# a-ludi/dentist

Hardware: AMD Instinct MI355X
Metric: gap-bases closed/sec (higher is better)
Workload: dtype u8

## Files before the change

dentist_amd/_lib.py:

```python
import ctypes
import os
import weakref

import numpy as np

_HERE = os.path.dirname(os.path.abspath(__file__))


def lib_path():
    return os.environ.get("DH_DEV_LIB") or os.path.join(_HERE, "libdentist_hip.so")


class DhError(RuntimeError):
    def __init__(self, code, msg):
        super().__init__(f"libdentist_hip error {code}: {msg}")
        self.code = code


class AlignOpts(ctypes.Structure):
    _fields_ = [(n, ctypes.c_int32) for n in (
        "k", "hmin", "band_shift", "tspace", "min_len", "pen", "xdrop", "max_err_ppm", "max_cand",
        "max_la", "tcap", "strands", "skip_self", "dmax", "width", "kmer_mod", "algo")]


# ... 29 lines not shown
    "contig_left", "status", "nreads", "ref_read", "ref_read_id", "crop_left", "crop_right", "left_aepos",
    "right_abpos", "ins_begin", "ins_end", "comp", "cons_len", "left_diffs", "right_diffs", "join")]
    + [("cons_off", "<i8"), ("contig_right", "<i4"), ("pad", "<i4")])

EXACT_HIT_DTYPE = np.dtype([("query", "<i4"), ("ref", "<i4"), ("begin", "<i8"), ("end", "<i8"), ("complement", "<i4"),
                            ("pad", "<i4")])

LA_DTYPE = np.dtype([("tlen", "<i4"), ("diffs", "<i4"), ("abpos", "<i4"), ("bbpos", "<i4"),
                     ("aepos", "<i4"), ("bepos", "<i4"), ("flags", "<u4"), ("aread", "<i4"),
                     ("bread", "<i4"), ("pad", "<i4"), ("toff", "<i8")])

SYMBOLS = [
    "dh_last_error", "dh_abi_version", "dh_ctx_create", "dh_ctx_destroy", "dh_ctx_sync",
    "dh_default_align_opts", "dh_db_create", "dh_db_destroy", "dh_db_drop_cache", "dh_db_nreads",
    "dh_db_total_bases", "dh_la_set_destroy", "dh_la_set_count", "dh_la_set_trace_len",
    "dh_la_set_records", "dh_la_set_trace", "dh_la_set_tspace", "dh_get_align_stats", "dh_get_cum_stats", "dh_get_mjoin_counts", "dh_get_join_counts", "dh_join_hit_capacity",
    "dh_ctx_release_scratch",
    "dh_align_db",
    "dh_las_write", "dh_las_read", "dh_default_process_opts", "dh_collect_spanning", "dh_pileups_destroy",
    "dh_pileups_count", "dh_pileups_get", "dh_process_pileups", "dh_insertions_destroy",
    "dh_insertions_count", "dh_insertions_records", "dh_insertions_bases", "dh_insertions_bases_len",
    "dh_get_process_stats", "dh_dazz_create_dam", "dh_dazz_create_db", "dh_dazz_split", "dh_dazz_open",
    "dh_dazz_close", "dh_dazz_nreads", "dh_dazz_first_id", "dh_dazz_bases", "dh_dazz_offsets",
    "dh_dazz_origin", "dh_dazz_fpulse", "dh_dazz_header", "dh_dazz_read_mask", "dh_dazz_write_mask",
    "dh_db_set_mask", "dh_output_fasta", "dh_tile_qv", "dh_consensus", "dh_las_merge",
    "dh_collect_candidates", "dh_pileups_create", "dh_pileups_select", "dh_align_db_block", "dh_la_set_merge",
    "dh_crop_pileups", "dh_cropped_create", "dh_cropped_destroy", "dh_cropped_npiles", "dh_cropped_records",
    "dh_cropped_nreads", "dh_cropped_pile", "dh_cropped_entry", "dh_cropped_read_id", "dh_cropped_offsets",
    "dh_cropped_bases", "dh_process_cropped", "dh_translate_trace_point", "dh_db_dust", "dh_db_get_mask",
    "dh_dazz_write_track", "dh_dazz_read_track", "dh_dazz_remove", "dh_dazz_flags",
    "dh_pileupdb_write", "dh_pileupdb_read", "dh_insertiondb_write", "dh_insertiondb_read", "dh_insertiondb_merge", "dh_chaindb_destroy",
# ... 255 lines not shown
        lib().dh_ctx_release_scratch.argtypes = [ctypes.c_void_p]
        _check(lib().dh_ctx_release_scratch(self._h))

    def mjoin_counts(self, reset=False):
        out = (ctypes.c_int64 * 2)()
        lib().dh_get_mjoin_counts.argtypes = [ctypes.c_void_p, ctypes.c_void_p, ctypes.c_int32]
        _check(lib().dh_get_mjoin_counts(self._h, out, int(reset)))
        return int(out[0]), int(out[1])

    def join_counts(self, reset=False):
        out = (ctypes.c_int64 * 4)()
        lib().dh_get_join_counts.argtypes = [ctypes.c_void_p, ctypes.c_void_p, ctypes.c_int32]
        _check(lib().dh_get_join_counts(self._h, out, int(reset)))
        return tuple(int(x) for x in out)

    def cum_stats(self, reset=False):
        st = CumStats()
        _check(lib().dh_get_cum_stats(self._h, ctypes.byref(st), int(reset)))
        return st

    def remap_skipping_reads(self, contigs, reads, contig_ids, read_ids, opts, allowance):
        ci = np.ascontiguousarray(contig_ids, dtype=np.int32)
        ri = np.ascontiguousarray(read_ids, dtype=np.int32)
        h = ctypes.c_void_p()
        L = lib()
        L.dh_remap_skipping_reads.argtypes = [ctypes.c_void_p, ctypes.c_void_p, ctypes.c_void_p, ctypes.c_void_p, ctypes.c_int32,
                                              ctypes.c_void_p, ctypes.c_int32, ctypes.c_void_p, ctypes.c_int32,
                                              ctypes.POINTER(ctypes.c_void_p)]
        _check(L.dh_remap_skipping_reads(self._h, contigs._h, reads._h, ci.ctypes.data, len(ci), ri.ctypes.data, len(ri),
                                         ctypes.byref(opts), int(allowance), ctypes.byref(h)))
# ... 1422 lines not shown
```

dentist_amd/csrc/dh_align.cpp:

```cpp
#include <chrono>
#include <cmath>
#include <cstdio>
#include <cstdlib>
#include <cstring>
#include <numeric>
#include <functional>
#include <memory>
#include <mutex>
#include <thread>

#include "dh_internal.h"
#include "dh_join.h"
#include "dh_mjoin.h"
#include "dh_tile.h"
#include "dh_parallel.h"

#define fail dh_fail

#ifdef DH_SEED_PROF
extern "C" void dhk_seed_prof_dump();
extern "C" void dhk_join_prof_dump();
extern "C" void dhk_tile_prof_dump();
#endif


extern "C" int dh_align_db(dh_ctx *ctx, dh_db *A, dh_db *B, const dh_align_opts *opts,
                           int32_t want_best, dh_la_set **out)
{
// ... 158 lines not shown
    }
    ~Tasks() { join(); }
};

struct AlignRun {
    dh_ctx *ctx;
    dh_db *A, *B;
    const dh_align_opts &o;
    int32_t first, count, want_best, want_sorted;
    const ChunkHook *hook;
    hipStream_t st;
    int32_t near_ppm;
    std::unique_ptr<dh_la_set> res, res2;
    Tasks tasks;
    dh_align_stats stats = {};
    bool tiled, use_join = false, use_mj = false, db_copies = false, want_packed = false, dual = false, sym_tiled = false,
         keep_dev = false;
    int64_t nitems_total, item_first, item_end;
    int32_t sepv = 0, chunk = 0, cn = 0, nbmax = 0, trmax = 0, per_wave = 0, poolcap = 0, nslots = 0, tile_waves = 0;
    int cap = 0;
    double dens = 0;
    int64_t mj_min_bases = 0;
    DhOpts dopt;
    IndexView iv;
    DbView av, bv;
    JoinView jv = {};
    int64_t join_hits = 0;
    float ms_join = 0;
    unsigned int jhist[4] = {0, 0, 0, 0};
    DhCand *d_cand = nullptr;
    int32_t *d_ncand = nullptr, *d_nhits = nullptr, *d_status = nullptr, *d_cdj = nullptr, *d_ovf = nullptr, *d_regs = nullptr;
// ... 375 lines not shown
    }
    HIPCHK(hipEventElapsedTime(&r.ms_join, ctx->ev[6], ctx->ev[7]));
    if (getenv("DH_TRACE"))
        fprintf(stderr, "[join] hit buffer %lld (%.1f MB), %lld hits, %d attempt(s); %.4f hits per base per read of depth from now on\n",
                (long long)ctx->join_first_cap, (double)ctx->join_first_cap * sizeof(uint64_t) / 1048576.0, (long long)r.join_hits,
                attempt + 1, ctx->join_hit_rate);
    if (!r.use_join) {
        if (getenv("DH_TRACE")) fprintf(stderr, "[join] a slice overflowed its table: falling back to the k-mer directory\n");
        HIPCHK(hipMemsetAsync(r.d_status, 0, sizeof(int32_t), st));
        if (int rc = dh_build_index(A, o.k, r.sepv, o.kmer_mod, false)) return rc;
        r.iv = index_view(A);
    }
    return DH_OK;
}

static int plan_seeds(AlignRun &r)
{
    dh_db *A = r.A, *B = r.B;
    const dh_align_opts &o = r.o;
    r.dens = (double)A->ix.n * std::max(1, o.kmer_mod) / std::pow(4.0, o.k) / std::max(1, A->ngroups);
    const double exp_hits = (double)B->max_len / std::max(1, o.kmer_mod) * (2.0 * r.dens + 0.1);
    int cap = 1024;
    while (cap < 16384 && exp_hits * 1.5 >= cap) cap *= 2;
    if (A == B) {
        cap = 1024;
        while (cap < 8192 && 0.6 * B->max_len > cap) cap *= 2;
    }
    if (r.use_join) {
        const unsigned int tol = (unsigned int)(0.3 * B->n);
        cap = r.jhist[0] <= tol ? 2048 : (r.jhist[1] <= tol ? 4096 : (r.jhist[2] <= tol ? 8192 : 16384));
    }
    if (const char *e = getenv("DH_SEED_CAP")) cap = atoi(e);
    r.cap = cap;
    r.use_mj = !r.use_join && A != B && !A->d_group && A->ngroups == 1 && !B->d_group && o.k >= MJ_MINK && o.k <= MJ_MAXK &&
               o.skip_self == 0 && r.want_packed && A->ix.n > 0 && A->ix.n < (1ll << 28) && !getenv("DH_NO_MJOIN");
    r.mj_min_bases = 64ll << 20;
    if (const char *e = getenv("DH_MJOIN_MIN")) r.mj_min_bases = atoll(e);
    if (r.use_mj && !A->ix.d_bitmap) {
        int32_t nbbits = std::min(MJ_MAXBITS, std::min(2 * o.k, std::max(MJ_PBITS + 5, dh_ceil_log2((uint64_t)A->ix.n) + 4)));
        const size_t words = (size_t)1 << (nbbits - 5);
        HIPCHK(dh_dev_alloc(&A->ix.d_bitmap, sizeof(uint32_t) * words));
        HIPCHK(dhk_memset(r.st, A->ix.d_bitmap, 0, sizeof(uint32_t) * words));
        dhk_mj_bitmap(r.st, A->ix.d_ent, A->ix.n, o.k, nbbits, A->ix.d_bitmap);
        HIPCHK(hipGetLastError());
        A->ix.nbbits = nbbits;
    }
    return DH_OK;
}

static int plan_mj_chunk(AlignRun &r, AlignChunk &c)
{
    dh_ctx *ctx = r.ctx;
    const dh_db *A = r.A, *B = r.B;
    const dh_align_opts &o = r.o;
    MjView &mv = c.mv;
    const int32_t cr0 = (int32_t)(c.item0 >> 1), cr1 = (int32_t)((c.item0 + c.ni) >> 1);
    const int64_t cb0 = B->h_off[(size_t)cr0], cb1 = B->h_off[(size_t)cr1];
    if (!r.use_mj || r.mj_skip_chunk || cb1 - cb0 < r.mj_min_bases || cb1 - cb0 >= (1ll << 40)) return DH_OK;
    mv.c0 = cb0;
    mv.c1 = cb1;
// ... 106 lines not shown
        SCR(SLOT_FSCR, d_fscr, (size_t)ctx->ncu * DH_SEED_FSCR_BLOCKS_PER_CU * DH_SEED_FSCR_WORDS)
    JoinView jv_mj = {};
    bool mj_chunk = false;
    if (c.mj_planned && !c.cc.has_n) {
        const MjView &mv = c.mv;
        HIPCHK(dhk_memset(st, mv.segtab, 0, sizeof(unsigned long long) * (size_t)(mv.r1 - mv.r0) * mv.nseg));
        dhk_mj_run(st, r.bv, r.iv, r.dopt, mv, ctx->ncu);
        HIPCHK(hipGetLastError());
        jv_mj.segtab = (uint64_t *)mv.segtab;
        jv_mj.hits = mv.rhits;
        jv_mj.status = r.d_status;
        jv_mj.ns_fixed = mv.nseg;
        jv_mj.read0 = mv.r0;
        mj_chunk = true;
    }
    const bool jn = r.use_join || mj_chunk;
    const JoinView &jvx = mj_chunk ? jv_mj : r.jv;
    const int tier_max = getenv("DH_SEED_NO16K") ? 8192 : 16384;
    const double kmers_per_read = (double)(B->h_off[(size_t)((item0 + ni) >> 1)] - B->h_off[(size_t)(item0 >> 1)]) /
                                  std::max(1, ni / 2) / std::max(1, o.kmer_mod);
    const double mean_hits = kmers_per_read * (2.0 * r.dens + 0.075);
    const bool wave_tier = mj_chunk && ctx->seed_wave_tier && 1.5 * mean_hits <= 512.0 && !getenv("DH_SEED_NO_WAVE_TIER");
    int capj = std::min(std::max(r.cap, 2048), tier_max);
    if (mj_chunk) {
        capj = 2048;
        while (capj < tier_max && 1.5 * mean_hits > capj) capj *= 2;
        if (wave_tier) capj = 512;
    }
    if (jn && capj > 4096) SCR(SLOT_FSCR, d_fscr, (size_t)ctx->ncu * DH_SEED_FSCR_BLOCKS_PER_CU * (capj > 8192 ? DH_SEED_FSCR_WORDS16 : DH_SEED_FSCR_WORDS))
    if (jn)
        dhk_seed_join(st, capj, r.bv, r.iv, r.dopt, jvx, (int32_t)item0, ni, c.candbase, c.ncandbase, c.nhitsbase, r.d_status,
                      r.d_queue + 1, ctx->ncu, d_fscr, nullptr, 0);
    else
        dhk_seed(st, r.cap, r.bv, r.iv, r.dopt, (int32_t)item0, ni, c.candbase, c.ncandbase, c.nhitsbase, r.d_status,
                 r.d_queue + 1, ctx->ncu, d_fscr);
    HIPCHK(hipGetLastError());
    int32_t status = 0;
    unsigned long long sm[4] = {0, 0, 0, 0};
    dhk_seed_summary(st, r.d_ncand, r.d_nhits, ni, r.d_summary);
// ... 42 lines not shown
        ctx->seed_wave_tier = 0;
        if (getenv("DH_TRACE"))
            fprintf(stderr, "[seeds] %zu of %d reads overflow the wavefront-per-read tier: not used by this context any more\n", big.size(), ni / 2);
    }
    size_t redo_all = (size_t)ni / 50 + 8;
    if (r.cap >= 8192) redo_all = (size_t)ni / 4;
    if (const char *e = getenv("DH_SEED_BIG_PCT")) redo_all = (size_t)((double)ni * atof(e) / 200.0);
    if (getenv("DH_TRACE") && !big.empty())
        fprintf(stderr, "[seeds] cap %d: %zu of %d reads overflow (whole chunk again above %zu)\n", r.cap, big.size(), ni / 2, redo_all);
    if (!jn && big.size() > redo_all && r.cap < 16384) {
        r.cap *= 2;
        *redo = true;
        return DH_OK;
    }
    if (mj_chunk) ctx->mj_chunks++;
    r.mj_skip_chunk = false;
    if (jn && capj < tier_max && !big.empty()) {
        std::vector<int32_t> huge;
        int32_t gcap2 = 0;
        for (int tier = capj < 2048 ? 2048 : 8192; tier <= tier_max; tier = tier < 8192 ? 8192 : tier * 2) {
            if (tier <= capj) continue;
            std::vector<int32_t> mid;
            huge.clear();
            gcap2 = 0;
            for (int32_t rd : big) {
                const size_t it = (size_t)(2 * (int64_t)rd - item0);
                const int32_t nh = r.h_nhits[it] + r.h_nhits[it + 1];
                if (nh <= tier)
                    mid.push_back(rd);
                else {
// ... 523 lines not shown
```

dentist_amd/csrc/dh_api.cpp:

```cpp
#include <cstring>

#include "dh_internal.h"

static_assert(sizeof(dh_align_opts) == sizeof(DhOpts), "opts layout");
static_assert(sizeof(dh_la) == sizeof(DhLa), "la layout");
static_assert(sizeof(dh_la) == 48, "la size");

static thread_local std::string g_err;

int dh_fail(int code, const std::string &msg)
{
    g_err = msg;
    return code;
}
#define fail dh_fail

extern "C" const char *dh_last_error(void) { return g_err.c_str(); }
extern "C" int32_t dh_abi_version(void) { return 4; }



extern "C" int dh_ctx_create(int32_t device, void *stream, dh_ctx **out)
{
    if (!out) return fail(DH_EINVAL, "dh_ctx_create: out is NULL");
// ... 104 lines not shown
{
    if (!c) return fail(DH_EINVAL, "ctx is NULL");
    HIPCHK(hipStreamSynchronize(c->stream));
    return DH_OK;
}

extern "C" int dh_get_mjoin_counts(dh_ctx *c, int64_t *out2, int32_t reset)
{
    if (!c || !out2) return fail(DH_EINVAL, "dh_get_mjoin_counts: NULL");
    out2[0] = c->mj_chunks;
    out2[1] = c->mj_fallbacks;
    if (reset) c->mj_chunks = c->mj_fallbacks = 0;
    return DH_OK;
}

extern "C" int dh_get_join_counts(dh_ctx *c, int64_t *out4, int32_t reset)
{
    if (!c || !out4) return fail(DH_EINVAL, "dh_get_join_counts: NULL");
    out4[0] = c->join_launches;
    out4[1] = c->join_reruns;
    out4[2] = c->join_last_hits;
    out4[3] = c->join_first_cap;
    if (reset) c->join_launches = c->join_reruns = c->join_last_hits = c->join_first_cap = 0;
    return DH_OK;
}

extern "C" int dh_get_align_stats(dh_ctx *c, dh_align_stats *out)
{
    if (!c || !out) return fail(DH_EINVAL, "dh_get_align_stats: NULL");
    *out = c->stats;
// ... 32 lines not shown
```

dentist_amd/csrc/dh_db.cpp:

```cpp
#include <cmath>
#include <cstdlib>

#include "dh_internal.h"

#define fail dh_fail


int dh_alloc_bases(hipStream_t st, int64_t total, uint8_t **alloc, uint8_t **base, bool pads_only)
{
    const size_t nb = (size_t)std::max<int64_t>(total, 0) + 2 * DB_PAD;
    HIPCHK(dh_dev_alloc(alloc, nb));
    if (pads_only) {
        HIPCHK(hipMemsetAsync(*alloc, 4, DB_PAD, st));
        HIPCHK(hipMemsetAsync(*alloc + nb - DB_PAD, 4, DB_PAD, st));
    } else
        HIPCHK(dhk_memset(st, *alloc, 4, nb));
    *base = *alloc + DB_PAD;
    return DH_OK;
}



extern "C" int dh_db_create(dh_ctx *ctx, const uint8_t *bases, const int64_t *off, int32_t n,
                            const int32_t *group, dh_db **out)
// ... 459 lines not shown
    HIPCHK(hipStreamSynchronize(ctx->stream));
    if (total != (unsigned long long)nent || total >= (1ull << 32) - 16)
        return fail(DH_EOVERFLOW, "index: more than 2^32 indexed k-mers (32-bit bucket offsets); raise kmer_mod");
    ix.n = (int64_t)nent;
    HIPCHK(dh_dev_alloc(&ix.d_ent, sizeof(ulonglong2) * (size_t)std::max<int64_t>(ix.n, 1)));
    if (gi_slices > 0)
        dhk_group_index(ctx->stream, 1, av, d_tiles, d_gtile, A->ngroups, gi_slices, gi_slice, k, kmer_mod, ix.shift,
                        ix.d_dir, ix.d_ent, ix.d_goff);
    else
        dhk_kmer_pass(ctx->stream, 1, av, d_tiles, (int32_t)tiles.size(), k, kmer_mod, ix.shift, ix.d_dir, ix.d_ent,
                      ix.d_goff);
    HIPCHK(hipGetLastError());
    HIPCHK(dh_dev_alloc(&ix.d_fat, sizeof(ulonglong2) * (size_t)nb));
    dhk_fat_dir(ctx->stream, ix.d_dir, ix.d_ent, nb, ix.d_fat);
    HIPCHK(hipGetLastError());
    HIPCHK(hipStreamSynchronize(ctx->stream));
    dh_dev_free(d_tiles);
    dh_dev_free(d_sums);
    dh_dev_free(ix.d_dir_alloc);
    ix.d_dir_alloc = ix.d_dir = nullptr;
    A->has_ix = true;
    return DH_OK;
}
```

dentist_amd/csrc/dh_internal.h:

```cpp
#ifndef DH_INTERNAL_H
#define DH_INTERNAL_H

#include "../../include/dentist_hip.h"

#include <hip/hip_runtime.h>

#include <algorithm>
#include <string>
#include <new>
#include <utility>
#include <vector>

#include "dh_device.h"

#define DB_PAD 64
#define PK_PAD 128

hipError_t dh_dev_alloc(void **p, size_t bytes);
void dh_dev_free(void *p);
void dh_dev_trim();
template <typename T>
inline hipError_t dh_dev_alloc(T **p, size_t bytes)
{
    return dh_dev_alloc((void **)p, bytes);
// ... 34 lines not shown
            return dh_fail(DH_EHIP, std::string(#expr) + ": " + hipGetErrorString(e_));          \
    } while (0)

enum DhSlot : int {
    SLOT_STATUS,
    SLOT_CAND, SLOT_NCAND, SLOT_NHITS, SLOT_NLA, SLOT_NTR, SLOT_POOL, SLOT_CDJ, SLOT_QUEUE, SLOT_LA, SLOT_TRSLOTS,
    SLOT_COUNTERS, SLOT_SUMS, SLOT_SUMMARY, SLOT_OVF, SLOT_REGS, SLOT_COLD, SLOT_LAOUT, SLOT_TROUT,
    SLOT_FSCR, SLOT_MID_LIST, SLOT_BIG_LIST, SLOT_BIG_HITS,
    SLOT_UNITS, SLOT_CANDOFF, SLOT_RECLIST, SLOT_RECCUR,
    SLOT_LA2, SLOT_TRSLOTS2, SLOT_NLA2, SLOT_NTR2, SLOT_A_PLANES, SLOT_A_RC_PLANES, SLOT_B_PK2, SLOT_B_RC_PK2, SLOT_LAOUT2,
    SLOT_TROUT2,
    SLOT_CHUNK_RC, SLOT_CHUNK_PK, SLOT_CHUNK_RCPK,
    SLOT_JOIN_BLOB, SLOT_JOIN_PSUB, SLOT_JOIN_ENTRIES, SLOT_JOIN_SEGTAB, SLOT_JOIN_CURSOR, SLOT_JOIN_HITS,
    SLOT_MJ_ENT, SLOT_MJ_SEGOFF, SLOT_MJ_TILE_N, SLOT_MJ_TILE_R, SLOT_MJ_SEG, SLOT_MJ_HSEG, SLOT_MJ_HITS, SLOT_MJ_RHITS,
    SLOT_MJ_SEGTAB, SLOT_MJ_CTR,
    SLOT_PR_VOFF, SLOT_PR_VOTES, SLOT_PR_OUT, SLOT_PR_STATUS, SLOT_PR_STAGE, SLOT_PR_SEGS, SLOT_PR_DECISIONS, SLOT_PR_CDIFF,
    SLOT_COMM_SEND, SLOT_COMM_RECV,
    SLOT_EP_TILES, SLOT_EP_DM, SLOT_EP_OW, SLOT_EP_RES, SLOT_EP_GEN_TILES, SLOT_EP_GEN_DM, SLOT_EP_GEN_OW, SLOT_EP_GEN_OFF,
    SLOT_EP_GEN_RES, SLOT_EP_COPY, SLOT_EP_OPS,
    SLOT_TR_RECS, SLOT_TR_BOUND, SLOT_TR_PAIRS, SLOT_TR_STATUS,
    SLOT_NW_REF, SLOT_NW_QRY, SLOT_NW_PAIRS, SLOT_NW_DM, SLOT_NW_OW, SLOT_NW_RES, SLOT_NW_COPY, SLOT_NW_OPS,
    SLOT_NWA_REF, SLOT_NWA_QRY, SLOT_NWA_PAIRS, SLOT_NWA_DM, SLOT_NWA_OW, SLOT_NWA_RES, SLOT_NWA_COPY, SLOT_NWA_OPS,
    SLOT_LOC_TEXT, SLOT_LOC_STARTS, SLOT_LOC_PW, SLOT_LOC_PATS, SLOT_LOC_MEMB, SLOT_LOC_TABLE, SLOT_LOC_BITMAP, SLOT_LOC_SHORTS,
    SLOT_LOC_CANDS, SLOT_LOC_COUNTER, SLOT_LOC_UNITS,
    DH_SLOT_COUNT
};
enum { DH_STW_STATUS = 0, DH_STW_PACK = 1, DH_STW_PACK_RC = 2, DH_STW_COUNT = 4 };
static_assert(DH_STW_PACK_RC == DH_STW_PACK + 1, "chunk_copies clears the two flag words with one memset");

#define DH_JOIN_HIT_RATE0 0.0128
#define DH_JOIN_HIT_MARGIN 1.5
#define DH_JOIN_HIT_MEM_FRACTION 0.25

struct dh_ctx {
    int device = 0;
    hipStream_t stream = nullptr;
    bool own_stream = false;
    int ncu = 0;
    hipEvent_t ev[8] = {};
    hipStream_t cstream = nullptr;
    hipEvent_t cev[4] = {};
    dh_align_stats stats = {};
    dh_cum_stats cum = {};
    double mj_hit_frac = 0.2;
    int seed_wave_tier = 1;
    int64_t mj_chunks = 0, mj_fallbacks = 0;
    double join_hit_rate = DH_JOIN_HIT_RATE0;
    int64_t join_launches = 0, join_reruns = 0, join_last_hits = 0, join_first_cap = 0;
    int32_t near_best_ppm = -1;
    dh_ctx *sub[3] = {nullptr, nullptr, nullptr};
    struct Arena {
        void *p = nullptr;
        size_t cap = 0;
    } arena[DH_SLOT_COUNT];
};
int dh_scratch(dh_ctx *ctx, DhSlot id, size_t bytes, void **out);
int dh_db_set_pflags(struct dh_db *db, const uint8_t *flags);

struct dh_index {
    uint32_t *d_dir = nullptr, *d_dir_alloc = nullptr;
    ulonglong2 *d_fat = nullptr;
    ulonglong2 *d_ent = nullptr;
    int64_t *d_goff = nullptr;
    int32_t *d_page_seq = nullptr;
    int64_t n = 0;
    int32_t k = 0, sepv = 0, shift = 0, pbits = 0, na = 0, kmer_mod = 1;
    uint32_t *d_bitmap = nullptr;
    int32_t nbbits = 0;
    bool light = false;
    void release()
    {
        dh_dev_free(d_dir_alloc);
        d_dir_alloc = nullptr;
        dh_dev_free(d_ent);
        dh_dev_free(d_goff);
        dh_dev_free(d_fat);
        d_fat = nullptr;
        dh_dev_free(d_page_seq);
        d_page_seq = nullptr;
        dh_dev_free(d_bitmap);
        d_bitmap = nullptr;
        nbbits = 0;
        d_dir = nullptr;
        d_ent = nullptr;
        d_goff = nullptr;
    }
// ... 127 lines not shown
```

dentist_amd/csrc/dh_process.cpp:

```cpp
#include <array>
#include <chrono>
#include <thread>
#include <cstdio>
#include <cstdlib>
#include <cstring>
#include <map>
#include <mutex>
#include <numeric>

#include "dh_internal.h"
#include "dh_parallel.h"

extern "C" {
void dhk_gather_slices(hipStream_t st, const uint8_t *src, const int64_t *src_off, const int32_t *sidx,
                       const int32_t *sbeg, const int64_t *dst_off, int32_t n, int32_t max_len,
                       uint8_t *dst);
void dhk_gather_parts(hipStream_t st, const uint8_t *src0, const int64_t *off0, const uint8_t *src1,
                      const int64_t *off1, const void *parts, int32_t n, int32_t max_len, uint8_t *dst);
void dhk_gather_ranges16(hipStream_t st, const uint16_t *src, const int64_t *desc, int32_t n, uint16_t *dst);
void dhk_tile_qv(hipStream_t st, const DhLa *las, const uint16_t *trace, const int32_t *la_first,
                 const int64_t *roff, int32_t nreads, int32_t tspace, const int32_t *cov, int32_t maxtiles,
                 uint8_t *qv);
void dhk_pile_funnel(hipStream_t st, DhLa *las, const uint32_t *item_off, int32_t nreads, const int64_t *roff,
                     int32_t max_err_ppm, int32_t tsp, int32_t *la_first, int32_t *live, int32_t *status);
// ... 1676 lines not shown
        rcs[0] = dh_fail(DH_EINVAL, std::string("dh_process_pileups: the first part of the batch failed: ") + e.what());
    }
    for (std::thread &w : workers) w.join();
    for (int32_t k = 1; k < nparts; k++) {
        dh_cum_stats &a = ctx->cum, &b = ctx->sub[k - 1]->cum;
        a.ms_index += b.ms_index; a.ms_seed += b.ms_seed; a.ms_wave += b.ms_wave; a.ms_gather += b.ms_gather;
        a.wave_launches += b.wave_launches; a.wave_cells += b.wave_cells; a.alignments += b.alignments; a.las += b.las;
        a.aligned_bp += b.aligned_bp; a.trace_values += b.trace_values; a.hits += b.hits; a.b_bases += b.b_bases;
        b = dh_cum_stats();
        dh_ctx *sc = ctx->sub[k - 1];
        ctx->join_launches += sc->join_launches;
        ctx->join_reruns += sc->join_reruns;
        ctx->join_last_hits += sc->join_last_hits;
        ctx->join_first_cap += sc->join_first_cap;
        sc->join_launches = sc->join_reruns = sc->join_last_hits = sc->join_first_cap = 0;
    }
    for (int32_t k = 0; k < nparts; k++)
        if (rcs[(size_t)k]) {
            for (dh_insertions *r : res) dh_insertions_destroy(r);
            if (k == 0) return rcs[0];
            return dh_fail(rcs[(size_t)k], msgs[(size_t)k].empty() ? "dh_process_pileups: a concurrent part of the batch failed" : msgs[(size_t)k]);
        }
    for (int32_t k = 1; k < nparts; k++) {
        for (int i = 0; i < 7; i++) g_pstats.ms[i] = std::max(g_pstats.ms[i], sts[(size_t)k].ms[i]);
        for (int i = 0; i < 3; i++) g_pstats.counters[i] += sts[(size_t)k].counters[i];
        for (int i = 0; i < 4; i++) g_pstats.work[i] += sts[(size_t)k].work[i];
    }
    dh_insertions *r0 = res[0];
    for (int32_t k = 1; k < nparts; k++) {
        dh_insertions *r1 = res[(size_t)k];
// ... 1267 lines not shown
```

include/dentist_hip.h:

```cpp
#ifndef DENTIST_HIP_H
#define DENTIST_HIP_H

#include <stddef.h>
#include <stdint.h>

#ifdef __cplusplus
extern "C" {
#endif

#define DH_OK 0
#define DH_EINVAL (-1)
#define DH_ENODEV (-2)
#define DH_EHIP (-3)
#define DH_EOVERFLOW (-4)
#define DH_EIO (-5)
#define DH_ENOMEM (-6)

const char *dh_last_error(void);
int32_t dh_abi_version(void);

typedef struct dh_ctx dh_ctx;
int dh_ctx_create(int32_t device, void *stream, dh_ctx **out);
void dh_ctx_destroy(dh_ctx *ctx);
int dh_ctx_sync(dh_ctx *ctx);
// ... 57 lines not shown
    float ms_index, ms_seed, ms_wave, ms_gather, ms_total;
    int32_t wave_launches;
    int32_t overflow_items;
    int64_t big_items;
} dh_align_stats;
int dh_get_align_stats(dh_ctx *ctx, dh_align_stats *out);

typedef struct {
    double ms_index, ms_seed, ms_wave, ms_gather;
    int64_t wave_launches, wave_cells, alignments, las, aligned_bp, trace_values, hits, b_bases;
} dh_cum_stats;
int dh_get_cum_stats(dh_ctx *ctx, dh_cum_stats *out, int32_t reset);
int dh_ctx_release_scratch(dh_ctx *ctx);
int dh_get_mjoin_counts(dh_ctx *ctx, int64_t *out2, int32_t reset);
int dh_get_join_counts(dh_ctx *ctx, int64_t *out4, int32_t reset);
int64_t dh_join_hit_capacity(const int64_t *bases, const int32_t *reads, int32_t ngroups, int32_t skip_self, double rate,
                             int64_t free_bytes);

int dh_align_db(dh_ctx *ctx, dh_db *A, dh_db *B, const dh_align_opts *opts, int32_t select_best,
                dh_la_set **out);
void dh_set_near_best(int32_t ppm);
int dh_ctx_set_near_best(dh_ctx *ctx, int32_t ppm);

int dh_align_db_block(dh_ctx *ctx, dh_db *A, dh_db *B, int32_t first, int32_t count,
                      const dh_align_opts *opts, int32_t select_best, dh_la_set **out);
int dh_align_db_transposed(dh_ctx *ctx, dh_db *A, dh_db *B, const dh_align_opts *opts, int32_t want_best,
                           dh_la_set **out, dh_la_set **out_transposed);
int dh_la_set_merge(const dh_la_set *const *sets, int32_t nsets, dh_la_set **out);

int dh_las_write(const char *path, const dh_la *las, int64_t n, const uint16_t *trace,
// ... 391 lines not shown
```

Baseline: 2.369 million.

## Add shared-memory hash-table join for grouped seed lookup

Adds a new seeding path (table join) for reads grouped by contig. For each group it builds a shared-memory hash table of the group's index k-mers, and each wave of B reads probes that table with count and write passes, producing segmented hit lists. It replaces the generic k-mer directory lookup when limits on group size, k and read length hold, and falls back otherwise. The cost is an extra count pass, a host sync per chunk to size the hit buffer with possible reruns, and an extra group-offset kernel at index build.

```diff
diff --git a/dentist_amd/_lib.py b/dentist_amd/_lib.py
--- a/dentist_amd/_lib.py
+++ b/dentist_amd/_lib.py
@@ -67,7 +67,7 @@
     "dh_last_error", "dh_abi_version", "dh_ctx_create", "dh_ctx_destroy", "dh_ctx_sync",
     "dh_default_align_opts", "dh_db_create", "dh_db_destroy", "dh_db_drop_cache", "dh_db_nreads",
     "dh_db_total_bases", "dh_la_set_destroy", "dh_la_set_count", "dh_la_set_trace_len",
-    "dh_la_set_records", "dh_la_set_trace", "dh_la_set_tspace", "dh_get_align_stats", "dh_get_cum_stats", "dh_get_mjoin_counts", "dh_get_join_counts", "dh_join_hit_capacity",
+    "dh_la_set_records", "dh_la_set_trace", "dh_la_set_tspace", "dh_get_align_stats", "dh_get_cum_stats", "dh_get_mjoin_counts", "dh_get_join_counts", "dh_get_tjoin_counts", "dh_join_hit_capacity",
     "dh_ctx_release_scratch",
     "dh_align_db",
     "dh_las_write", "dh_las_read", "dh_default_process_opts", "dh_collect_spanning", "dh_pileups_destroy",
@@ -353,6 +353,12 @@
         _check(lib().dh_get_join_counts(self._h, out, int(reset)))
         return tuple(int(x) for x in out)
 
+    def tjoin_counts(self, reset=False):
+        out = (ctypes.c_int64 * 4)()
+        lib().dh_get_tjoin_counts.argtypes = [ctypes.c_void_p, ctypes.c_void_p, ctypes.c_int32]
+        _check(lib().dh_get_tjoin_counts(self._h, out, int(reset)))
+        return tuple(int(x) for x in out)
+
     def cum_stats(self, reset=False):
         st = CumStats()
         _check(lib().dh_get_cum_stats(self._h, ctypes.byref(st), int(reset)))
diff --git a/dentist_amd/csrc/dh_align.cpp b/dentist_amd/csrc/dh_align.cpp
--- a/dentist_amd/csrc/dh_align.cpp
+++ b/dentist_amd/csrc/dh_align.cpp
@@ -12,6 +12,7 @@
 #include "dh_internal.h"
 #include "dh_join.h"
 #include "dh_mjoin.h"
+#include "dh_tjoin.h"
 #include "dh_tile.h"
 #include "dh_parallel.h"
 
@@ -200,7 +201,7 @@
     std::unique_ptr<dh_la_set> res, res2;
     Tasks tasks;
     dh_align_stats stats = {};
-    bool tiled, use_join = false, use_mj = false, db_copies = false, want_packed = false, dual = false, sym_tiled = false,
+    bool tiled, use_join = false, use_mj = false, use_tj = false, db_copies = false, want_packed = false, dual = false, sym_tiled = false,
          keep_dev = false;
     int64_t nitems_total, item_first, item_end;
     int32_t sepv = 0, chunk = 0, cn = 0, nbmax = 0, trmax = 0, per_wave = 0, poolcap = 0, nslots = 0, tile_waves = 0;
@@ -606,6 +607,11 @@
     return DH_OK;
 }
 
+static void ctx_count_tj_fallback(dh_ctx *ctx)
+{
+    ctx->tj_fallbacks++;
+    if (getenv("DH_TRACE")) fprintf(stderr, "[tjoin] a limit of the table join is not met: this call keeps the k-mer directory\n");
+}
 static int plan_seeds(AlignRun &r)
 {
     dh_db *A = r.A, *B = r.B;
@@ -636,6 +642,17 @@
         dhk_mj_bitmap(r.st, A->ix.d_ent, A->ix.n, o.k, nbbits, A->ix.d_bitmap);
         HIPCHK(hipGetLastError());
         A->ix.nbbits = nbbits;
+    }
+    if (!r.use_join && A != B && A->d_group && !getenv("DH_NO_TJOIN")) {
+        int64_t tcap_ent = TJ_CAP;
+        if (const char *e = getenv("DH_TJOIN_CAP")) tcap_ent = std::max<int64_t>(0, std::min<int64_t>(TJ_CAP, atoll(e)));
+        r.use_tj = B->d_group && o.k <= TJ_MAXK && o.skip_self == 0 && A->ix.d_gent &&
+                   A->ix.max_gent <= tcap_ent && A->ix.n < (1ll << 31) && B->max_len < (1 << 24);
+        if (!r.use_tj) ctx_count_tj_fallback(r.ctx);
+        if (r.use_tj) {
+            r.ctx->tj_calls++;
+            r.ctx->tj_last_hits = 0;
+        }
     }
     return DH_OK;
 }
@@ -772,15 +789,82 @@
         jv_mj.read0 = mv.r0;
         mj_chunk = true;
     }
-    const bool jn = r.use_join || mj_chunk;
-    const JoinView &jvx = mj_chunk ? jv_mj : r.jv;
+    JoinView jv_tj = {};
+    bool tj_chunk = false;
+    unsigned long long tj_hits = 0;
+    if (r.use_tj) {
+        const int32_t cr0 = (int32_t)(item0 >> 1), cr1 = (int32_t)((item0 + ni) >> 1);
+        std::vector<int4> units;
+        for (int32_t rd = cr0; rd < cr1;) {
+            const int32_t g = B->h_group[(size_t)rd];
+            int32_t e = rd + 1;
+            while (e < cr1 && e - rd < TJ_RUN && B->h_group[(size_t)e] == g) e++;
+            units.push_back(int4{g, rd, e, 0});
+            rd = e;
+        }
+        const int64_t cbases = B->h_off[(size_t)cr1] - B->h_off[(size_t)cr0];
+        int64_t hcap = (int64_t)(1.25 * ctx->tj_hit_rate * (double)cbases) + 4096;
+        if (const char *e = getenv("DH_TJOIN_HITCAP")) hcap = std::max<int64_t>(1, atoll(e));
+        TjView tv = {};
+        int4 *d_units;
+        uint32_t *d_tjctr;
+        SCR(SLOT_TJ_UNITS, d_units, units.size())
+        SCR(SLOT_TJ_SEGTAB, tv.segtab, (size_t)(cr1 - cr0))
+        SCR(SLOT_TJ_CTR, d_tjctr, 4)
+        HIPCHK(hipMemcpyAsync(d_units, units.data(), sizeof(int4) * units.size(), hipMemcpyHostToDevice, st));
+        tv.gent = r.A->ix.d_gent;
+        tv.ngroups = r.A->ngroups;
+        tv.units = d_units;
+        tv.nunits = (int32_t)units.size();
+        tv.read0 = cr0;
+        tv.cursor = (unsigned long long *)d_tjctr;
+        tv.queue = d_tjctr + 2;
+        tv.status = r.d_status;
+        int32_t tst = 0;
+        for (int attempt = 0;; attempt++) {
+            SCR(SLOT_TJ_HITS, tv.hits, (size_t)hcap)
+            tv.hits_cap = hcap;
+            HIPCHK(hipMemsetAsync(d_tjctr, 0, 4 * sizeof(uint32_t), st));
+            dhk_tjoin(st, r.bv, r.iv, r.dopt, tv, ctx->ncu);
+            HIPCHK(hipGetLastError());
+            HIPCHK(hipMemcpyAsync(&tj_hits, tv.cursor, sizeof(tj_hits), hipMemcpyDeviceToHost, st));
+            HIPCHK(hipMemcpyAsync(&tst, r.d_status, sizeof(int32_t), hipMemcpyDeviceToHost, st));
+            HIPCHK(hipStreamSynchronize(st));
+            if (!(tst & DH_ST_TJ_HITCAP)) break;
+            if (attempt > 0) return fail(DH_EOVERFLOW, "table join: the hit buffer sized by the count pass was too small");
+            tst &= ~DH_ST_TJ_HITCAP;
+            HIPCHK(hipMemcpyAsync(r.d_status, &tst, sizeof(int32_t), hipMemcpyHostToDevice, st));
+            if (getenv("DH_TRACE")) fprintf(stderr, "[tjoin] hit buffer of %lld too small for %llu hits: run again\n", (long long)hcap, tj_hits);
+            hcap = (int64_t)tj_hits;
+            ctx->tj_reruns++;
+        }
+        if (cbases > 0) ctx->tj_hit_rate = std::max(DH_TJ_HIT_RATE0, (double)tj_hits / (double)cbases);
+        if (tst & DH_ST_TJ_OVERFLOW) {
+            tst &= ~DH_ST_TJ_OVERFLOW;
+            HIPCHK(hipMemcpyAsync(r.d_status, &tst, sizeof(int32_t), hipMemcpyHostToDevice, st));
+            HIPCHK(hipStreamSynchronize(st));
+            r.use_tj = false;
+            ctx->tj_calls--;
+            ctx_count_tj_fallback(ctx);
+            *redo = true;
+            return DH_OK;
+        }
+        jv_tj.segtab = tv.segtab;
+        jv_tj.hits = tv.hits;
+        jv_tj.status = r.d_status;
+        jv_tj.ns_fixed = 1;
+        jv_tj.read0 = cr0;
+        tj_chunk = true;
+    }
+    const bool jn = r.use_join || mj_chunk || tj_chunk;
+    const JoinView &jvx = mj_chunk ? jv_mj : (tj_chunk ? jv_tj : r.jv);
     const int tier_max = getenv("DH_SEED_NO16K") ? 8192 : 16384;
     const double kmers_per_read = (double)(B->h_off[(size_t)((item0 + ni) >> 1)] - B->h_off[(size_t)(item0 >> 1)]) /
                                   std::max(1, ni / 2) / std::max(1, o.kmer_mod);
-    const double mean_hits = kmers_per_read * (2.0 * r.dens + 0.075);
-    const bool wave_tier = mj_chunk && ctx->seed_wave_tier && 1.5 * mean_hits <= 512.0 && !getenv("DH_SEED_NO_WAVE_TIER");
+    const double mean_hits = tj_chunk ? (double)tj_hits / std::max(1, ni / 2) : kmers_per_read * (2.0 * r.dens + 0.075);
+    const bool wave_tier = (mj_chunk || tj_chunk) && ctx->seed_wave_tier && 1.5 * mean_hits <= 512.0 && !getenv("DH_SEED_NO_WAVE_TIER");
     int capj = std::min(std::max(r.cap, 2048), tier_max);
-    if (mj_chunk) {
+    if (mj_chunk || tj_chunk) {
         capj = 2048;
         while (capj < tier_max && 1.5 * mean_hits > capj) capj *= 2;
         if (wave_tier) capj = 512;
@@ -853,6 +937,7 @@
         return DH_OK;
     }
     if (mj_chunk) ctx->mj_chunks++;
+    if (tj_chunk) ctx->tj_last_hits += (int64_t)tj_hits;
     r.mj_skip_chunk = false;
     if (jn && capj < tier_max && !big.empty()) {
         std::vector<int32_t> huge;
diff --git a/dentist_amd/csrc/dh_api.cpp b/dentist_amd/csrc/dh_api.cpp
--- a/dentist_amd/csrc/dh_api.cpp
+++ b/dentist_amd/csrc/dh_api.cpp
@@ -142,6 +142,17 @@
     return DH_OK;
 }
 
+extern "C" int dh_get_tjoin_counts(dh_ctx *c, int64_t *out4, int32_t reset)
+{
+    if (!c || !out4) return fail(DH_EINVAL, "dh_get_tjoin_counts: NULL");
+    out4[0] = c->tj_calls;
+    out4[1] = c->tj_fallbacks;
+    out4[2] = c->tj_last_hits;
+    out4[3] = c->tj_reruns;
+    if (reset) c->tj_calls = c->tj_fallbacks = c->tj_last_hits = c->tj_reruns = 0;
+    return DH_OK;
+}
+
 extern "C" int dh_get_join_counts(dh_ctx *c, int64_t *out4, int32_t reset)
 {
     if (!c || !out4) return fail(DH_EINVAL, "dh_get_join_counts: NULL");
diff --git a/dentist_amd/csrc/dh_db.cpp b/dentist_amd/csrc/dh_db.cpp
--- a/dentist_amd/csrc/dh_db.cpp
+++ b/dentist_amd/csrc/dh_db.cpp
@@ -2,6 +2,7 @@
 #include <cstdlib>
 
 #include "dh_internal.h"
+#include "dh_tjoin.h"
 
 #define fail dh_fail
 
@@ -497,7 +498,16 @@
     HIPCHK(dh_dev_alloc(&ix.d_fat, sizeof(ulonglong2) * (size_t)nb));
     dhk_fat_dir(ctx->stream, ix.d_dir, ix.d_ent, nb, ix.d_fat);
     HIPCHK(hipGetLastError());
+    std::vector<uint32_t> gent;
+    if (A->d_group && ix.shift <= 2 * k) {
+        gent.resize((size_t)A->ngroups + 1);
+        HIPCHK(dh_dev_alloc(&ix.d_gent, sizeof(uint32_t) * gent.size()));
+        dhk_tj_group_offsets(ctx->stream, ix.d_dir, A->ngroups, k, ix.shift, nb, ix.d_gent);
+        HIPCHK(hipGetLastError());
+        HIPCHK(hipMemcpyAsync(gent.data(), ix.d_gent, sizeof(uint32_t) * gent.size(), hipMemcpyDeviceToHost, ctx->stream));
+    }
     HIPCHK(hipStreamSynchronize(ctx->stream));
+    for (size_t g2 = 0; g2 + 1 < gent.size(); g2++) ix.max_gent = std::max<int64_t>(ix.max_gent, (int64_t)gent[g2 + 1] - (int64_t)gent[g2]);
     dh_dev_free(d_tiles);
     dh_dev_free(d_sums);
     dh_dev_free(ix.d_dir_alloc);
diff --git a/dentist_amd/csrc/dh_internal.h b/dentist_amd/csrc/dh_internal.h
--- a/dentist_amd/csrc/dh_internal.h
+++ b/dentist_amd/csrc/dh_internal.h
@@ -72,6 +72,7 @@
     SLOT_JOIN_BLOB, SLOT_JOIN_PSUB, SLOT_JOIN_ENTRIES, SLOT_JOIN_SEGTAB, SLOT_JOIN_CURSOR, SLOT_JOIN_HITS,
     SLOT_MJ_ENT, SLOT_MJ_SEGOFF, SLOT_MJ_TILE_N, SLOT_MJ_TILE_R, SLOT_MJ_SEG, SLOT_MJ_HSEG, SLOT_MJ_HITS, SLOT_MJ_RHITS,
     SLOT_MJ_SEGTAB, SLOT_MJ_CTR,
+    SLOT_TJ_UNITS, SLOT_TJ_SEGTAB, SLOT_TJ_HITS, SLOT_TJ_CTR,
     SLOT_PR_VOFF, SLOT_PR_VOTES, SLOT_PR_OUT, SLOT_PR_STATUS, SLOT_PR_STAGE, SLOT_PR_SEGS, SLOT_PR_DECISIONS, SLOT_PR_CDIFF,
     SLOT_COMM_SEND, SLOT_COMM_RECV,
     SLOT_EP_TILES, SLOT_EP_DM, SLOT_EP_OW, SLOT_EP_RES, SLOT_EP_GEN_TILES, SLOT_EP_GEN_DM, SLOT_EP_GEN_OW, SLOT_EP_GEN_OFF,
@@ -89,6 +90,8 @@
 #define DH_JOIN_HIT_RATE0 0.0128
 #define DH_JOIN_HIT_MARGIN 1.5
 #define DH_JOIN_HIT_MEM_FRACTION 0.25
+
+#define DH_TJ_HIT_RATE0 0.14
 
 struct dh_ctx {
     int device = 0;
@@ -103,6 +106,8 @@
     double mj_hit_frac = 0.2;
     int seed_wave_tier = 1;
     int64_t mj_chunks = 0, mj_fallbacks = 0;
+    int64_t tj_calls = 0, tj_fallbacks = 0, tj_last_hits = 0, tj_reruns = 0;
+    double tj_hit_rate = DH_TJ_HIT_RATE0;
     double join_hit_rate = DH_JOIN_HIT_RATE0;
     int64_t join_launches = 0, join_reruns = 0, join_last_hits = 0, join_first_cap = 0;
     int32_t near_best_ppm = -1;
@@ -126,8 +131,13 @@
     uint32_t *d_bitmap = nullptr;
     int32_t nbbits = 0;
     bool light = false;
+    uint32_t *d_gent = nullptr;
+    int64_t max_gent = 0;
     void release()
     {
+        dh_dev_free(d_gent);
+        d_gent = nullptr;
+        max_gent = 0;
         dh_dev_free(d_dir_alloc);
         d_dir_alloc = nullptr;
         dh_dev_free(d_ent);
diff --git a/dentist_amd/csrc/dh_process.cpp b/dentist_amd/csrc/dh_process.cpp
--- a/dentist_amd/csrc/dh_process.cpp
+++ b/dentist_amd/csrc/dh_process.cpp
@@ -1714,6 +1714,11 @@
         ctx->join_last_hits += sc->join_last_hits;
         ctx->join_first_cap += sc->join_first_cap;
         sc->join_launches = sc->join_reruns = sc->join_last_hits = sc->join_first_cap = 0;
+        ctx->tj_calls += sc->tj_calls;
+        ctx->tj_fallbacks += sc->tj_fallbacks;
+        ctx->tj_last_hits += sc->tj_last_hits;
+        ctx->tj_reruns += sc->tj_reruns;
+        sc->tj_calls = sc->tj_fallbacks = sc->tj_last_hits = sc->tj_reruns = 0;
     }
     for (int32_t k = 0; k < nparts; k++)
         if (rcs[(size_t)k]) {
diff --git a/dentist_amd/csrc/dh_tjoin.h b/dentist_amd/csrc/dh_tjoin.h
--- /dev/null
+++ b/dentist_amd/csrc/dh_tjoin.h
@@ -0,0 +1,86 @@
+#ifndef DH_TJOIN_H
+#define DH_TJOIN_H
+#include <stdint.h>
+
+#if defined(__HIPCC__)
+#define TJ_HD __host__ __device__ __forceinline__
+#else
+#define TJ_HD inline
+#endif
+
+#define TJ_SLOT_BITS 14
+#define TJ_SLOTS (1 << TJ_SLOT_BITS)
+#define TJ_CAP 8192
+#define TJ_THREADS 1024
+#define TJ_RUN (TJ_THREADS / 64)
+#define TJ_QBATCH 4
+#define TJ_MAXK 16
+#define TJ_EMPTY (~0ull)
+
+#define DH_ST_TJ_HITCAP 0x80
+#define DH_ST_TJ_OVERFLOW 0x100
+
+TJ_HD uint32_t tj_home(uint32_t canon) { return (canon * 0x9E3779B1u) >> (32 - TJ_SLOT_BITS); }
+TJ_HD uint64_t tj_slot(uint32_t canon, uint32_t ori, uint32_t idx) { return ((uint64_t)canon << 32) | (ori << 31) | idx; }
+
+template <class Claim>
+TJ_HD void tj_insert(uint64_t *tab, uint64_t v, Claim claim)
+{
+    uint32_t h = tj_home((uint32_t)(v >> 32));
+    while (!claim(tab + h, v)) h = (h + 1) & (TJ_SLOTS - 1);
+}
+
+template <class F>
+TJ_HD void tj_walk(const uint64_t *tab, uint32_t canon, F f)
+{
+    for (uint32_t h = tj_home(canon);; h = (h + 1) & (TJ_SLOTS - 1)) {
+        const uint64_t s = tab[h];
+        if (s == TJ_EMPTY) return;
+        if ((uint32_t)(s >> 32) == canon) f((uint32_t)s);
+    }
+}
+
+struct TjMatch {
+    int32_t fwd, rev;
+    uint32_t emit;
+};
+TJ_HD TjMatch tj_match(const uint64_t *tab, uint32_t canon, uint32_t bori, bool pal, int32_t tcap, int32_t strands)
+{
+    int32_t runf = 0, runr = 0;
+    tj_walk(tab, canon, [&](uint32_t lo) {
+        const bool same = (lo >> 31) == bori;
+        runf += (same || pal) ? 1 : 0;
+        runr += (!same || pal) ? 1 : 0;
+    });
+    TjMatch m;
+    m.emit = ((runf > 0 && runf <= tcap && (strands & 1)) ? 1u : 0u) | ((runr > 0 && runr <= tcap && (strands & 2)) ? 2u : 0u);
+    m.fwd = (m.emit & 1u) ? runf : 0;
+    m.rev = (m.emit & 2u) ? runr : 0;
+    return m;
+}
+
+#ifndef DH_TJOIN_SLOT_CODE_ONLY
+#include "dh_device.h"
+#include "dh_join.h"
+
+struct TjView {
+    const uint32_t *gent;
+    int32_t ngroups;
+    const int4 *units;
+    int32_t nunits;
+    int32_t read0;
+    uint64_t *segtab;
+    uint64_t *hits;
+    int64_t hits_cap;
+    unsigned long long *cursor;
+    uint32_t *queue;
+    int32_t *status;
+};
+
+extern "C" {
+void dhk_tj_group_offsets(hipStream_t st, const uint32_t *dir, int32_t ngroups, int32_t k, int32_t shift, int64_t nb,
+                          uint32_t *gent);
+void dhk_tjoin(hipStream_t st, DbView B, IndexView ix, DhOpts o, TjView t, int32_t ncu);
+}
+#endif
+#endif
diff --git a/dentist_amd/csrc/dh_tjoin.hip b/dentist_amd/csrc/dh_tjoin.hip
--- /dev/null
+++ b/dentist_amd/csrc/dh_tjoin.hip
@@ -0,0 +1,225 @@
+#include <hip/hip_runtime.h>
+#include <stdint.h>
+#include <stdio.h>
+#include <stdlib.h>
+
+#include <algorithm>
+
+#include "dh_kmer.h"
+#include "dh_tjoin.h"
+
+#define LANES 64
+#define HIT_QBITS 24
+
+#ifdef DH_TJ_PROF
+__device__ unsigned long long g_tj_prof[4];
+#define TP(i) if (tid == 0) { const unsigned long long t_ = wall_clock64(); atomicAdd(&g_tj_prof[i], t_ - tp_); tp_ = t_; }
+#define TP_BEGIN unsigned long long tp_ = wall_clock64();
+extern "C" void dhk_tj_prof_dump()
+{
+    unsigned long long h[4];
+    (void)hipMemcpyFromSymbol(h, HIP_SYMBOL(g_tj_prof), sizeof(h));
+    if (h[3])
+        fprintf(stderr, "[tj prof] k_tjoin, %llu units: table build %.1f roll + probe %.1f write %.1f us per unit and block\n", h[3],
+                h[0] / 100.0 / h[3], h[1] / 100.0 / h[3], h[2] / 100.0 / h[3]);
+    unsigned long long z[4] = {0};
+    (void)hipMemcpyToSymbol(HIP_SYMBOL(g_tj_prof), z, sizeof(z));
+}
+#else
+#define TP(i)
+#define TP_BEGIN
+#endif
+
+__global__ void __launch_bounds__(256)
+k_tj_group_offsets(const uint32_t *__restrict__ dir, int32_t ngroups, int32_t k, int32_t shift, int64_t nb, uint32_t *__restrict__ gent)
+{
+    const int32_t g = blockIdx.x * blockDim.x + threadIdx.x;
+    if (g > ngroups) return;
+    int64_t b = (int64_t)(((uint64_t)g << (2 * k)) >> shift);
+    b = b < nb ? b : nb;
+    gent[g] = dir[b - 1];
+}
+
+static __device__ __forceinline__ uint32_t tj_pack8(uint64_t w)
+{
+    uint64_t x = __builtin_bswap64(w) & 0x0303030303030303ull;
+    x = (x | (x >> 6)) & 0x000F000F000F000Full;
+    x = (x | (x >> 12)) & 0x000000FF000000FFull;
+    return (uint32_t)((x | (x >> 24)) & 0xFFFFull);
+}
+
+template <bool WRITE>
+static __device__ uint32_t tj_read(const DbView &B, const IndexView &ix, const DhOpts &o, const KmerSampler &smp, const uint64_t *tab,
+                                   int32_t r, int lane, uint32_t g0, uint64_t *__restrict__ out, uint32_t limit, uint32_t *cur)
+{
+    constexpr int PER = 8, STEP = LANES * PER;
+    constexpr uint64_t BAD = 0xFCFCFCFCFCFCFCFCull;
+    const int64_t bo = B.off[r];
+    const int32_t blen = (int32_t)(B.off[r + 1] - bo);
+    const uint8_t *b = B.bases + bo;
+    const int k = o.k;
+    const int32_t npos = blen - k + 1;
+    const uint32_t kmask = k >= 16 ? 0xFFFFFFFFu : ((1u << (2 * k)) - 1u);
+    const uint32_t kbits = (1u << k) - 1u;
+    uint32_t cnt = 0;
+    uint64_t n0 = 0, n1 = 0, n2 = 0, nm = 0;
+    auto fetch = [&](int32_t q0) {
+        if (q0 < npos) {
+            n0 = load8(b + q0);
+            n1 = load8(b + q0 + 8);
+            n2 = load8(b + q0 + 16);
+            if (B.mask_bits) nm = load8(B.mask_bits + ((bo + q0) >> 3)) >> ((bo + q0) & 7);
+        }
+    };
+    fetch(lane * PER);
+    for (int32_t base = 0; base < npos; base += STEP) {
+        const int32_t q0 = base + lane * PER;
+        const uint64_t w0 = n0, w1 = n1, w2 = n2;
+        const uint32_t mbits = (uint32_t)nm;
+        fetch(q0 + STEP);
+        if (q0 >= npos) continue;
+        uint32_t nbits = 0;
+        if ((w0 | w1 | w2) & BAD) {
+            for (int i = 0; i < 8; i++) {
+                nbits |= (((w0 >> (8 * i)) & 0xFC) ? 1u : 0u) << i;
+                nbits |= (((w1 >> (8 * i)) & 0xFC) ? 1u : 0u) << (8 + i);
+                nbits |= (((w2 >> (8 * i)) & 0xFC) ? 1u : 0u) << (16 + i);
+            }
+        }
+        const uint64_t P = ((uint64_t)tj_pack8(w0) << 32) | ((uint64_t)tj_pack8(w1) << 16) | (uint64_t)tj_pack8(w2);
+        uint64_t R = __brevll(~P);
+        R = (((R >> 1) & 0x5555555555555555ull) | ((R & 0x5555555555555555ull) << 1)) >> 16;
+#pragma unroll
+        for (int j = 0; j < PER; j++) {
+            const int32_t q = q0 + j;
+            const uint32_t km = (uint32_t)(P >> (48 - 2 * k - 2 * j)) & kmask;
+            const uint32_t rc = (uint32_t)(R >> (2 * j)) & kmask;
+            const uint32_t canon = km < rc ? km : rc;
+            const bool em = q < npos && !(((nbits | mbits) >> j) & kbits) && kmer_sampled((uint64_t)canon, smp);
+            if (!em) continue;
+            const uint32_t bori = km != canon ? 1u : 0u;
+            const bool pal = km == rc;
+            const TjMatch m = tj_match(tab, canon, bori, pal, o.tcap, o.strands);
+            if (!WRITE)
+                cnt += (uint32_t)(m.fwd + m.rev);
+            else if (m.emit) {
+                tj_walk(tab, canon, [&](uint32_t lo) {
+                    const bool same = (lo >> 31) == bori;
+                    const int64_t gv = (int64_t)(ix.ent[g0 + (lo & 0x7FFFFFFFu)].y & ((1ull << 40) - 1));
+                    for (int32_t strand = 0; strand < 2; strand++) {
+                        if (!(m.emit & (1u << strand)) || !(strand ? (!same || pal) : (same || pal))) continue;
+                        const int32_t qs = strand ? blen - k - q : q;
+                        const int64_t D = gv + ix.sepv - qs;
+                        const uint32_t slot = atomicAdd(cur, 1u);
+                        if (slot < limit) out[slot] = ((uint64_t)strand << 63) | ((uint64_t)D << HIT_QBITS) | (uint32_t)qs;
+                        cnt++;
+                    }
+                });
+            }
+        }
+    }
+    return cnt;
+}
+
+__global__ void __launch_bounds__(TJ_THREADS, 1)
+k_tjoin(DbView B, IndexView ix, DhOpts o, TjView t)
+{
+    __shared__ uint64_t tab[TJ_SLOTS];
+    __shared__ uint32_t s_cnt[TJ_RUN], s_cur[TJ_RUN];
+    __shared__ unsigned long long s_base;
+    __shared__ int32_t s_work, s_ok;
+    const int tid = threadIdx.x, lane = tid & (LANES - 1), wv = tid / LANES;
+    const KmerSampler smp = kmer_sampler(o.kmer_mod, o.k);
+    const uint64_t kmask = (1ull << (2 * o.k)) - 1;
+    int32_t have = -1;
+    uint32_t g0 = 0;
+    TP_BEGIN
+    for (;;) {
+        __syncthreads();
+        if (tid == 0) s_work = (int32_t)atomicAdd(t.queue, (uint32_t)TJ_QBATCH);
+        __syncthreads();
+        const int32_t u0 = s_work;
+        if (u0 >= t.nunits) break;
+#pragma unroll 1
+        for (int32_t u = u0; u < min(u0 + TJ_QBATCH, t.nunits); u++) {
+            const int4 un = t.units[u];
+            if (un.x != have) {
+                have = un.x;
+                uint32_t g1 = 0;
+                g0 = 0;
+                if ((uint32_t)un.x < (uint32_t)t.ngroups) {
+                    g0 = t.gent[un.x];
+                    g1 = t.gent[un.x + 1];
+                }
+                if (g1 - g0 > (uint32_t)TJ_CAP || g1 > (uint32_t)ix.n || g1 < g0) {
+                    if (tid == 0) atomicOr(t.status, DH_ST_TJ_OVERFLOW);
+                    g1 = g0;
+                }
+                for (int32_t i = tid; i < TJ_SLOTS; i += TJ_THREADS) tab[i] = TJ_EMPTY;
+                __syncthreads();
+                for (uint32_t e = g0 + tid; e < g1; e += TJ_THREADS) {
+                    const uint64_t x = ix.ent[e].x;
+                    tj_insert(tab, tj_slot((uint32_t)(x & kmask), (uint32_t)(x >> 63), e - g0), [](uint64_t *p, uint64_t v) {
+                        return atomicCAS((unsigned long long *)p, (unsigned long long)TJ_EMPTY, (unsigned long long)v) == TJ_EMPTY;
+                    });
+                }
+                __syncthreads();
+                TP(0)
+            }
+            const int32_t r = un.y + wv;
+            const bool mine = r < un.z;
+            uint32_t c = mine ? tj_read<false>(B, ix, o, smp, tab, r, lane, g0, nullptr, 0u, nullptr) : 0u;
+            for (int off = LANES / 2; off > 0; off >>= 1) c += __shfl_xor(c, off, LANES);
+            if (lane == 0) {
+                s_cnt[wv] = c;
+                s_cur[wv] = 0;
+            }
+            __syncthreads();
+            if (tid == 0) {
+                unsigned long long total = 0;
+                for (int i = 0; i < TJ_RUN; i++) total += s_cnt[i];
+                const unsigned long long base = total ? atomicAdd(t.cursor, total) : 0ull;
+                const bool ok = base + total <= (unsigned long long)t.hits_cap;
+                if (!ok) atomicOr(t.status, DH_ST_TJ_HITCAP);
+                s_base = base;
+                s_ok = ok ? 1 : 0;
+            }
+            __syncthreads();
+            TP(1)
+            if (mine && s_ok) {
+                unsigned long long first = s_base;
+                for (int i = 0; i < wv; i++) first += s_cnt[i];
+                if (c >= (1u << 24) || first >= (1ull << 40)) {
+                    if (lane == 0) atomicOr(t.status, DH_ST_TJ_OVERFLOW);
+                } else {
+                    if (c) tj_read<true>(B, ix, o, smp, tab, r, lane, g0, t.hits + first, c, &s_cur[wv]);
+                    if (lane == 0) t.segtab[r - t.read0] = (first << 24) | c;
+                }
+            }
+            __syncthreads();
+            TP(2)
+#ifdef DH_TJ_PROF
+            if (tid == 0) atomicAdd(&g_tj_prof[3], 1ull);
+#endif
+        }
+    }
+}
+
+extern "C" void dhk_tj_group_offsets(hipStream_t st, const uint32_t *dir, int32_t ngroups, int32_t k, int32_t shift, int64_t nb,
+                                     uint32_t *gent)
+{
+    hipLaunchKernelGGL(k_tj_group_offsets, dim3((unsigned)((ngroups + 1 + 255) / 256)), dim3(256), 0, st, dir, ngroups, k, shift, nb, gent);
+}
+
+extern "C" void dhk_tjoin(hipStream_t st, DbView B, IndexView ix, DhOpts o, TjView t, int32_t ncu)
+{
+    if (t.nunits <= 0) return;
+    const int32_t batches = (t.nunits + TJ_QBATCH - 1) / TJ_QBATCH;
+    hipLaunchKernelGGL(k_tjoin, dim3((unsigned)std::min(batches, std::max(1, ncu))), dim3(TJ_THREADS), 0, st, B, ix, o, t);
+#ifdef DH_TJ_PROF
+    if (getenv("DH_TRACE")) {
+        (void)hipStreamSynchronize(st);
+        dhk_tj_prof_dump();
+    }
+#endif
+}
diff --git a/include/dentist_hip.h b/include/dentist_hip.h
--- a/include/dentist_hip.h
+++ b/include/dentist_hip.h
@@ -95,6 +95,7 @@
 int dh_ctx_release_scratch(dh_ctx *ctx);
 int dh_get_mjoin_counts(dh_ctx *ctx, int64_t *out2, int32_t reset);
 int dh_get_join_counts(dh_ctx *ctx, int64_t *out4, int32_t reset);
+int dh_get_tjoin_counts(dh_ctx *ctx, int64_t *out4, int32_t reset);
 int64_t dh_join_hit_capacity(const int64_t *bases, const int32_t *reads, int32_t ngroups, int32_t skip_self, double rate,
                              int64_t free_bytes);
 
```

After: 2.419 million, median of 6. 1.02x the previous value.
